# y00njaekim/CMU-11785-IDL-1.58bit-ASR

Hardware: AMD Instinct MI355X
Metric: mel-frames/sec (Conformer-S 1.58-bit train step) (higher is better)
Workload: dtype fp32; 1 GPU; conformer-s-1.58bit-train-step; global_batch=32, execution=hip-graph, per_gpu_batch=32, frames=1000, d_model=144, blocks=16, d_ff=576, heads=4, vocab=5004, parallelism=dp1, passes=teacher 2-bit + student 1-bit + SP, conv_pointwise=fp32 (reference)

## Files before the change

cmu-11785-idl-1.58bit-asr_amd/csrc/capi.hip:

```cpp
#include <float.h>

#include <algorithm>
#include <vector>

#include "../../include/onebit_hip.h"
#include "ob_launch.h"
#include <stdint.h>

using namespace ob;

namespace {

constexpr int kAbiVersion = 4;

inline hipStream_t as_stream(void* s) { return reinterpret_cast<hipStream_t>(s); }

inline bool aligned4(const void* p) { return (reinterpret_cast<uintptr_t>(p) & 3) == 0; }
inline bool misaligned8(const void* p) { return (reinterpret_cast<uintptr_t>(p) & 7) != 0; }

inline int check_bits(int bits) { return (bits == 1 || bits == 2) ? OB_OK : OB_ERR_BITWIDTH; }

inline int launched() {
  const hipError_t e = hipGetLastError();
  return e == hipSuccess ? OB_OK : OB_ERR_HIP;
// ... 2090 lines not shown
    return OB_ERR_NULL;
  if (((uintptr_t)saved & 15) || ((uintptr_t)probs & 15)) return OB_ERR_ALIGN;
  launch_relattn_fwd(q, k, v, pos, u, vb, lens, Bt, P, T, H, d, p_drop,
                     reinterpret_cast<const uint64_t*>(rng), (uint64_t)rng_offset, saved, probs,
                     ctx, as_stream(stream));
  return launched();
}

int64_t ob_relattn_saved_elems(int64_t Bt, int64_t T, int64_t H, int64_t d) {
  if (Bt < 1 || H < 1 || !relattn_supported(T, d)) return 0;
  return relattn_saved_elems(Bt, T, H, d);
}

size_t ob_relattn_bwd_workspace(int64_t Bt, int64_t T, int64_t H, int64_t d) {
  if (Bt < 1 || H < 1 || !relattn_supported(T, d)) return 0;
  return align_up(relattn_bwd_workspace(Bt, T, H, d));
}

int ob_relattn_set_bwd_mode(int mode) { return relattn_set_flash(mode); }

int ob_tgemm_set_colloop(int on) { return tgemm_set_colloop(on); }

int ob_relattn_set_kv_ring(int on) { return relattn_set_kv_ring(on); }

int64_t ob_relattn_probs_elems(int64_t Bt, int64_t T, int64_t H) {
  if (Bt < 1 || H < 1 || T < 1) return 0;
  return relattn_probs_elems(Bt, T, H);
}

int ob_relattn_bwd(const float* dctx, const float* ctx, const float* q, const float* k,
                   const float* v, const float* pos, const float* u, const float* vb,
                   const int32_t* lens, int64_t Bt, int64_t P, int64_t T, int64_t H, int64_t d,
                   float p_drop, const int64_t* rng, int64_t rng_offset, const float* saved,
                   int64_t saved_elems, float* dq, float* dk, float* dv, float* dpos, float* du,
                   float* dvb, void* ws, size_t ws_bytes, void* stream) {
  if (int st = relattn_check(Bt, P, T, H, d, p_drop)) return st;
  if (!dctx || !ctx || !q || !k || !v || !pos || !u || !vb || !lens || !saved || !dq || !dk ||
      !dv || !dpos || !du || !dvb || !ws)
    return OB_ERR_NULL;
  if (saved_elems != relattn_saved_elems(Bt, T, H, d)) return OB_ERR_SHAPE;
  (void)rng;
  (void)rng_offset;
  if ((uintptr_t)saved & 15) return OB_ERR_ALIGN;
  if (ws_bytes < ob_relattn_bwd_workspace(Bt, T, H, d)) return OB_ERR_WORKSPACE;
  launch_relattn_bwd(dctx, ctx, q, k, v, pos, u, vb, lens, Bt, P, T, H, d, p_drop, saved, dq, dk,
                     dv, dpos, du, dvb, ws, as_stream(stream));
// ... 107 lines not shown
```

cmu-11785-idl-1.58bit-asr_amd/csrc/ob_launch.h:

```cpp
#pragma once

#include <hip/hip_runtime.h>
#include <stddef.h>
#include <stdint.h>

#include "../../include/onebit_hip.h"

namespace ob {

inline int64_t ceil_div(int64_t a, int64_t b) { return (a + b - 1) / b; }

void launch_quant_pack(const float* W, const float* alpha, int alpha_raw, int bits,
                       const int* bits_dev, int64_t N, int64_t K, uint32_t* codes,
                       uint32_t* codes_t, hipStream_t s);
int64_t quant_pack_item_blocks(int64_t N, int64_t K);
int64_t quant_pack_item_blocks16(int64_t N, int64_t K);
void launch_quant_pack_group(const ob_pack_item* items_dev, int n_items, int64_t total_blocks,
                             hipStream_t s);
void launch_quant_dequant(const float* W, const float* alpha, int alpha_raw, int bits, int64_t n,
                          float* W_hat, hipStream_t s);

int64_t ste_reduce_blocks(int64_t total);
void launch_ste_reduce(const float* part, int chunks, int64_t nk, const float* part_db,
                       int64_t n_db, const float* W, const float* alpha, int alpha_raw, int bits,
// ... 438 lines not shown
  float* param;
  const float* grad;
  float* exp_avg;
  float* exp_avg_sq;
  int64_t numel;
};
int64_t adamw_plan(const int64_t* numels, int64_t n, int64_t* map);
size_t adamw_workspace(int64_t n_blocks);
void launch_adamw(const AdamwTensor* tab, const int64_t* map, int64_t nb, const float* lr,
                  float* step, float grad_scale, double beta1, double beta2, double eps,
                  double weight_decay, double max_norm, float* total_norm_out, void* ws,
                  hipStream_t s);

bool embed_supported(int64_t C);
void launch_embed_bwd(const int64_t* idx, int64_t N, const float* g, int64_t C, int64_t V,
                      int64_t pad, float* dW, hipStream_t s);

bool relattn_supported(int64_t T, int64_t d);
size_t relattn_bwd_workspace(int64_t Bt, int64_t T, int64_t H, int64_t d);
int64_t relattn_probs_elems(int64_t Bt, int64_t T, int64_t H);
int64_t relattn_saved_elems(int64_t Bt, int64_t T, int64_t H, int64_t d);
int relattn_set_flash(int on);
int relattn_set_kv_ring(int on);
void launch_relattn_fwd(const float* q, const float* k, const float* v, const float* pos,
                        const float* u, const float* vb, const int* lens, int64_t Bt, int64_t P,
                        int64_t T, int64_t H, int64_t d, float p_drop, const uint64_t* rng,
                        uint64_t rng_off, float* saved, float* probs, float* ctx, hipStream_t s);
void launch_relattn_bwd(const float* dctx, const float* ctx, const float* q, const float* k,
                        const float* v, const float* pos, const float* u, const float* vb,
                        const int* lens, int64_t Bt, int64_t P, int64_t T, int64_t H, int64_t d,
                        float p_drop, const float* saved, float* dq, float* dk, float* dv,
                        float* dpos, float* du, float* dvb, void* ws, hipStream_t s);
void launch_relattn_dropout_mask(int64_t n, int64_t T, float p_drop, const uint64_t* rng,
                                 uint64_t rng_off, uint8_t* out, hipStream_t s);

bool subsample_supported(int64_t T, int64_t F, int64_t C);
size_t subsample_image_bytes(int64_t C);
void launch_subsample_pack(const float* W2, int64_t C, void* img, hipStream_t s);
void launch_subsample_fwd(const float* X, int64_t B, int64_t T, int64_t F, int64_t C,
                          const float* W0, const float* b0, const void* img, const float* b2,
                          float* Y1, float* Y2, hipStream_t s);
size_t subsample_bwd_workspace(int64_t B, int64_t T, int64_t F, int64_t C);
void launch_subsample_bwd(const float* X, const float* W0, const float* b0, const float* Y1,
                          const float* Y2, const float* dY2, int64_t B, int64_t T, int64_t F,
                          int64_t C, const void* img,
                          float* dW0, float* db0, float* dW2, float* db2, void* ws,
// ... 4 lines not shown
```

cmu-11785-idl-1.58bit-asr_amd/csrc/relattn.hip:

```cpp
#include <atomic>
#include <math.h>

#include <algorithm>

#include "ob_drop.h"
#include "ob_launch.h"
#include "ob_mma.h"

namespace {
template <typename F>
__device__ __forceinline__ uint32_t xrows_1632(uint32_t x, F op) {
  const auto a = __builtin_amdgcn_permlane16_swap(x, x, false, false);
  x = op(a[0], a[1]);
  const auto b = __builtin_amdgcn_permlane32_swap(x, x, false, false);
  return op(b[0], b[1]);
}
__device__ __forceinline__ float xsum_1632(float v) {
  return __builtin_bit_cast(float, xrows_1632(__builtin_bit_cast(uint32_t, v), [](uint32_t a, uint32_t b) {
    return __builtin_bit_cast(uint32_t, __builtin_bit_cast(float, a) + __builtin_bit_cast(float, b));
  }));
}
__device__ __forceinline__ float xmax_1632(float v) {
  return __builtin_bit_cast(float, xrows_1632(__builtin_bit_cast(uint32_t, v), [](uint32_t a, uint32_t b) {
    return __builtin_bit_cast(uint32_t, fmaxf(__builtin_bit_cast(float, a), __builtin_bit_cast(float, b)));
  }));
}
__device__ __forceinline__ uint32_t xor_1632(uint32_t v) {
  return xrows_1632(v, [](uint32_t a, uint32_t b) { return a | b; });
}
}

namespace ob {

namespace {

constexpr int kThreads = 256;
constexpr int kTile = 64;
constexpr int kFwdKeyChunk = 256;

__device__ __forceinline__ void split_pair(float x0, float x1, uint32_t (&w)[3]) {
  __bf16 h0, m0, l0, h1, m1, l1;
  split3(x0, h0, m0, l0);
  split3(x1, h1, m1, l1);
  w[0] = (uint32_t)__builtin_bit_cast(uint16_t, h0) | ((uint32_t)__builtin_bit_cast(uint16_t, h1) << 16);
  w[1] = (uint32_t)__builtin_bit_cast(uint16_t, m0) | ((uint32_t)__builtin_bit_cast(uint16_t, m1) << 16);
  w[2] = (uint32_t)__builtin_bit_cast(uint16_t, l0) | ((uint32_t)__builtin_bit_cast(uint16_t, l1) << 16);
}

typedef f32x4 f32x4u __attribute__((aligned(4)));
template <int N>
__device__ __forceinline__ void load_run(const float* __restrict__ p, float (&out)[N]) {
#pragma unroll
  for (int i = 0; i + 4 <= N; i += 4) {
    const f32x4 v = *(const f32x4u*)(p + i);
    out[i] = v[0];
    out[i + 1] = v[1];
    out[i + 2] = v[2];
    out[i + 3] = v[3];
  }
#pragma unroll
  for (int i = N & ~3; i < N; ++i) out[i] = p[i];
// ... 12 lines not shown
  return __builtin_amdgcn_make_buffer_rsrc(const_cast<float*>(base), (short)0,
                                           (int)(((size_t)(T - 1) * C + D) * sizeof(float)),
                                           0x00020000);
}

template <int DQ>
__device__ __forceinline__ void load_group_buf(__amdgpu_buffer_rsrc_t rs, int voff, int C, int t0,
                                               float (&dst)[4][DQ]) {
#pragma unroll
  for (int u = 0; u < 4; ++u) {
    const int soff = 64 * (t0 + u) * C;
#pragma unroll
    for (int i = 0; i + 4 <= DQ; i += 4) {
      const f32x4 v = __builtin_amdgcn_raw_buffer_load_b128(rs, voff + 4 * i, soff, 0);
      dst[u][i] = v[0];
      dst[u][i + 1] = v[1];
      dst[u][i + 2] = v[2];
      dst[u][i + 3] = v[3];
    }
#pragma unroll
    for (int i = DQ & ~3; i < DQ; ++i)
      dst[u][i] = __builtin_bit_cast(float, __builtin_amdgcn_raw_buffer_load_b32(rs, voff + 4 * i, soff, 0));
  }
}

struct BlockId {
  int qt, h, b;
};

__device__ __forceinline__ BlockId block_id(int nqt, int H) {
  const int L = xcd_logical((int)blockIdx.x, (int)gridDim.x);
  BlockId id;
  id.qt = L % nqt;
  const int rest = L / nqt;
  id.h = rest % H;
  id.b = rest / H;
  return id;
}

__device__ __forceinline__ size_t frag_off(int bh, int a, int t, int nt) {
  return (((size_t)bh * nt + a) * nt + t) * 256;
}

__device__ __forceinline__ uint64_t drop_row_base(int bh, int T, int i) {
  return ((uint64_t)bh * T + i) * (uint64_t)(T + (T & 1));
}
// ... 13 lines not shown
      st_acc[k] += st_n - st_t;                              \
      st_t = st_n;                                           \
    }                                                        \
  } while (0)
#define OB_STAMP_WRITE(NWV)                                                             \
  if constexpr (st_on) {                                                                \
    const uint64_t st_rt1 = __builtin_amdgcn_s_memrealtime();                           \
    const size_t st_w = (size_t)blockIdx.x * (NWV) + w;                                 \
    if (lane == 0 && st_w * 10 + 10 <= 65536)                                           \
      for (int k_ = 0; k_ < 10; ++k_) g_attn_stamps[st_w * 10 + k_] = st_acc[k_];       \
    if (lane == 0 && st_w * 2 + 2 <= 16384) {                                           \
      g_attn_rt[st_w * 2] = st_rt0;                                                     \
      g_attn_rt[st_w * 2 + 1] = st_rt1;                                                 \
    }                                                                                   \
  }
#else
#define OB_STAMP_DECL(K)
#define OB_STAMP(k) \
  do {              \
  } while (0)
#define OB_STAMP_WRITE(NWV)
#endif

template <int DQ, int NTT>
__global__ __launch_bounds__(kThreads) void relattn_fwd_kernel(
    const float* __restrict__ q, const float* __restrict__ k, const float* __restrict__ v,
    const float* __restrict__ pos, const float* __restrict__ u, const float* __restrict__ vbias,
    const int* __restrict__ lens, int Bp, int T, int H, float inv_sqrt_d, DropCfg dc,
    const uint64_t* __restrict__ rng, uint64_t rng_off, float* __restrict__ probs,
    float* __restrict__ stats, uint32_t* __restrict__ kbits, float* __restrict__ anchors,
    float* __restrict__ ctx) {
  constexpr int D = 4 * DQ;
  constexpr int CT = (D + 15) / 16;
  extern __shared__ float img[];
  const int nt = (T + 15) >> 4;
  const int ldi = T + 1;
  const BlockId bid = block_id((T + kTile - 1) / kTile, H);
  const int b = bid.b, h = bid.h, i0 = bid.qt * kTile;
  const int bh = b * H + h;
  const int pass = b / Bp;
  const int C = H * D;
  const int L = min(lens[b], T);
  const int lane = threadIdx.x & 63, w = threadIdx.x >> 6, r = lane & 15, g = lane >> 4;
  const float* qb = q + (size_t)b * T * C + h * D;
  const float* kb = k + (size_t)b * T * C + h * D;
  const float* vbp = v + (size_t)b * T * C + h * D;
  const float* pb = pos + (size_t)pass * T * C + h * D;
  const float* ub = u + h * D;
  const float* vbb = vbias + h * D;
  const __amdgpu_buffer_rsrc_t rs_p = slice_rsrc(pb, T, C, D), rs_k = slice_rsrc(kb, T, C, D);
  const int voff_a = (r * C + g * DQ) * 4;
  OB_STAMP_DECL(3)

  const int ir = 16 * w + r;
  const int qi = i0 + ir;
  const int qic = min(qi, T - 1);
  float qu[DQ], qv[DQ];
  {
    float x[DQ];
    load_run<DQ>(qb + (size_t)qic * C + g * DQ, x);
#pragma unroll
    for (int s = 0; s < DQ; ++s) {
      const int c = g * DQ + s;
      qu[s] = x[s] + ub[c];
      qv[s] = x[s] + vbb[c];
    }
  }

  float opb[2][4][DQ];
  load_group_buf<DQ>(rs_p, voff_a, C, 0, opb[0]);
  OB_STAMP(0);
#pragma unroll
  for (int t0 = 0; t0 < NTT; t0 += 4) {
    if (t0 >= nt) continue;
    float (&opa)[4][DQ] = opb[(t0 >> 2) & 1];
    if (t0 + 4 < NTT && t0 + 4 < nt) load_group_buf<DQ>(rs_p, voff_a, C, t0 + 4, opb[((t0 >> 2) + 1) & 1]);
    f32x4 acc[4];
#pragma unroll
    for (int uu = 0; uu < 4; ++uu) acc[uu] = f32x4{0.f, 0.f, 0.f, 0.f};
#pragma unroll
    for (int s = 0; s < DQ; ++s)
#pragma unroll
      for (int uu = 0; uu < 4; ++uu) acc[uu] = mfma4(opa[uu][s], qv[s], acc[uu]);
#pragma unroll
    for (int uu = 0; uu < 4; ++uu) {
      const int t = t0 + uu;
      if (t >= nt) continue;
      float* dst = img + ir * ldi + 1 + 16 * t + 4 * g;
      if (16 * t + 15 < T) {
#pragma unroll
        for (int j = 0; j < 4; ++j) dst[j] = acc[uu][j];
      } else {
#pragma unroll
        for (int j = 0; j < 4; ++j)
          if (16 * t + 4 * g + j < T) dst[j] = acc[uu][j];
      }
    }
  }
  if (g == 0) img[ir * ldi] = 0.0f;
  OB_STAMP(1);
  load_group_buf<DQ>(rs_k, voff_a, C, 0, opb[0]);
  if (i0 + kTile < T) {
    const float* qe = qb + (size_t)(i0 + kTile) * C;
    for (int m = threadIdx.x; m < T; m += kThreads) {
      float pr[D];
      load_run<D>(pb + (size_t)m * C, pr);
      float a = 0.0f;
#pragma unroll
      for (int c = 0; c < D; ++c) a = fmaf(qe[c] + vbb[c], pr[c], a);
      img[kTile * ldi + 1 + m] = a;
    }
    if (threadIdx.x == 0) img[kTile * ldi] = 0.0f;
  }
  OB_STAMP(2);
  __syncthreads();
  OB_STAMP(3);
  if (anchors) {
    const int nchk = (16 * nt + 31) / 32;
#pragma unroll
    for (int half = 0; half < 2; ++half) {
      const int row = i0 + 32 * half;
      if (row < 32 || row >= T) continue;
      float* dst = anchors + ((size_t)bh * nchk + row / 32 - 1) * T;
      for (int m = threadIdx.x; m < T; m += kThreads) dst[m] = img[32 * half * ldi + 1 + m];
    }
  }

  float sreg[NTT][4];
  float mx = -INFINITY;
  const float* bdp = img + (T + ir * T + 4 * g - i0);
  const int Lq = qi < L ? L : 0;
#pragma unroll
  for (int t0 = 0; t0 < NTT; t0 += 4) {
    if (t0 >= nt) continue;
    float (&opa)[4][DQ] = opb[(t0 >> 2) & 1];
    if (t0 + 4 < NTT && t0 + 4 < nt) load_group_buf<DQ>(rs_k, voff_a, C, t0 + 4, opb[((t0 >> 2) + 1) & 1]);
    f32x4 acc4[4];
#pragma unroll
    for (int uu = 0; uu < 4; ++uu) acc4[uu] = f32x4{0.f, 0.f, 0.f, 0.f};
#pragma unroll
    for (int s = 0; s < DQ; ++s)
#pragma unroll
      for (int uu = 0; uu < 4; ++uu) acc4[uu] = mfma4(opa[uu][s], qu[s], acc4[uu]);
#pragma unroll
    for (int uu = 0; uu < 4; ++uu) {
      const int t = t0 + uu;
      if (t >= nt) continue;
#pragma unroll
      for (int j = 0; j < 4; ++j) {
        const float sc = (acc4[uu][j] + bdp[16 * t + j]) * inv_sqrt_d;
        sreg[t][j] = 16 * t + 4 * g + j < Lq ? sc : -INFINITY;
        mx = fmaxf(mx, sreg[t][j]);
      }
    }
  }
  mx = xmax_1632(mx);
  OB_STAMP(4);
  constexpr int kVSlots = (kFwdKeyChunk / 2 * DQ + kThreads - 1) / kThreads;
  constexpr bool kVPre = DQ <= 9;
// ... 149 lines not shown
          for (int j = 0; j < 4; ++j) {
            bfr[p][j] = lo[j];
            bfr[p][4 + j] = hi[j];
          }
        }
        o[ct] = mfma_x6(af, bfr, o[ct]);
      }
    }
  }
#pragma unroll
  for (int ct = 0; ct < CT; ++ct) {
    const int col = 16 * ct + r;
    if (col >= D) continue;
#pragma unroll
    for (int j = 0; j < 4; ++j) {
      const int row = i0 + 16 * w + 4 * g + j;
      if (row < T) ctx[((size_t)b * T + row) * C + h * D + col] = o[ct][j];
    }
  }
  OB_STAMP(9);
  OB_STAMP_WRITE(kThreads / 64)
}

template <int DQ, int NTT>
__global__ __launch_bounds__(kThreads) void relattn_bwd_kernel(
    const float* __restrict__ dctx, const float* __restrict__ ctxo, const float* __restrict__ k,
    const float* __restrict__ v, const float* __restrict__ pos, int Bp, int T, int H,
    float inv_sqrt_d, DropCfg dc, const float* __restrict__ probs, float* __restrict__ dq,
    float* __restrict__ dsg, float* __restrict__ du_part, float* __restrict__ dvb_part) {
  constexpr int D = 4 * DQ;
  constexpr int CT = (D + 15) / 16;
  extern __shared__ float band[];
  __shared__ float red[kThreads / 64][2][64];
  const int nt = (T + 15) >> 4;
  const int nqt = (T + kTile - 1) / kTile;
  const BlockId bid = block_id(nqt, H);
  const int b = bid.b, h = bid.h, qt = bid.qt, i0 = qt * kTile;
  const int bh = b * H + h;
  const int pass = b / Bp;
  const int C = H * D;
  const int lane = threadIdx.x & 63, w = threadIdx.x >> 6, r = lane & 15, g = lane >> 4;
  const size_t bo = (size_t)b * T * C + h * D;
  const float* kb = k + bo;
  const float* vbp = v + bo;
  const float* dob = dctx + bo;
  const float* cob = ctxo + bo;
  const float* pb = pos + (size_t)pass * T * C + h * D;
  const __amdgpu_buffer_rsrc_t rs_v = slice_rsrc(vbp, T, C, D), rs_k = slice_rsrc(kb, T, C, D),
                               rs_p = slice_rsrc(pb, T, C, D);
  const int voff_a = (r * C + g * DQ) * 4;
  auto keep_scale = [&](float pv) -> float {
    if (!dc.on) return 1.0f;
    return __builtin_signbit(pv) ? 0.0f : dc.scale;
  };
  if (threadIdx.x < 128) band[(kTile + 1) * T + threadIdx.x] = 0.0f;
  OB_STAMP_DECL(2)

  const int ir = 16 * w + r;
  const int qi = i0 + ir;
  const int qic = min(qi, T - 1);
  float dor[DQ];
  load_run<DQ>(dob + (size_t)qic * C + g * DQ, dor);
  float delta;
  {
    float cr[DQ];
    load_run<DQ>(cob + (size_t)qic * C + g * DQ, cr);
    float a = 0.0f;
#pragma unroll
    for (int s = 0; s < DQ; ++s) a = fmaf(dor[s], cr[s], a);
    a = xsum_1632(a);
    delta = a;
  }
  OB_STAMP(0);

  const bool arow_ok = (i0 >> 4) + w < nt;
  const float* pf = probs + frag_off(bh, arow_ok ? (i0 >> 4) + w : 0, 0, nt) + 4 * lane;
  float* brow = band + (1 + ir) * T + 4 * g;
  float dsr[NTT][4];
  float opb[2][4][DQ];
  load_group_buf<DQ>(rs_v, voff_a, C, 0, opb[0]);
#pragma unroll
  for (int t0 = 0; t0 < NTT; t0 += 4) {
    if (t0 >= nt) continue;
    float (&opa)[4][DQ] = opb[(t0 >> 2) & 1];
    if (t0 + 4 < NTT && t0 + 4 < nt) load_group_buf<DQ>(rs_v, voff_a, C, t0 + 4, opb[((t0 >> 2) + 1) & 1]);
    f32x4 p4[4];
#pragma unroll
    for (int uu = 0; uu < 4; ++uu)
      p4[uu] = arow_ok && t0 + uu < nt ? *reinterpret_cast<const f32x4*>(pf + 256 * (t0 + uu))
                                       : f32x4{0.f, 0.f, 0.f, 0.f};
    f32x4 acc4[4];
#pragma unroll
    for (int uu = 0; uu < 4; ++uu) acc4[uu] = f32x4{0.f, 0.f, 0.f, 0.f};
#pragma unroll
    for (int s = 0; s < DQ; ++s)
#pragma unroll
      for (int uu = 0; uu < 4; ++uu) acc4[uu] = mfma4(opa[uu][s], dor[s], acc4[uu]);
#pragma unroll
    for (int uu = 0; uu < 4; ++uu) {
      const int t = t0 + uu;
      if (t >= nt) continue;
#pragma unroll
      for (int j = 0; j < 4; ++j) {
        const float pv = p4[uu][j];
        const float dp = acc4[uu][j] * keep_scale(pv);
        const float ds = (fabsf(pv) * (dp - delta)) * inv_sqrt_d;
        dsr[t][j] = ds;
      }
      if (16 * t + 15 < T) {
#pragma unroll
        for (int j = 0; j < 4; ++j) brow[16 * t + j] = dsr[t][j];
      } else {
#pragma unroll
        for (int j = 0; j < 4; ++j)
          if (16 * t + 4 * g + j < T) brow[16 * t + j] = dsr[t][j];
      }
    }
  }

  OB_STAMP(1);
  if (i0 > 0) {
    const int ip = i0 - 1;
    const float* drow = dob + (size_t)ip * C;
    const float* crow = cob + (size_t)ip * C;
    float dl = 0.0f;
#pragma unroll
    for (int c = 0; c < D; ++c) dl = fmaf(drow[c], crow[c], dl);
    const float* pr = probs + frag_off(bh, ip >> 4, 0, nt) + 4 * (ip & 15);
    for (int jj = threadIdx.x; jj < T; jj += kThreads) {
      float vr[D];
      load_run<D>(vbp + (size_t)jj * C, vr);
      float a = 0.0f;
#pragma unroll
      for (int c = 0; c < D; ++c) a = fmaf(vr[c], drow[c], a);
      const float pv = pr[256 * (jj >> 4) + 64 * ((jj & 15) >> 2) + (jj & 3)];
      band[jj] = (fabsf(pv) * (a * keep_scale(pv) - dl)) * inv_sqrt_d;
    }
  } else {
    for (int jj = threadIdx.x; jj < T; jj += kThreads) band[jj] = 0.0f;
  }
  OB_STAMP(2);

  f32x4 oq[CT];
#pragma unroll
  for (int ct = 0; ct < CT; ++ct) oq[ct] = f32x4{0.f, 0.f, 0.f, 0.f};
  const int voff_b = (4 * g * C + r) * 4;
  auto load_b = [&](int t, float (&dst)[4][CT]) {
#pragma unroll
    for (int j = 0; j < 4; ++j)
#pragma unroll
      for (int ct = 0; ct < CT; ++ct)
        dst[j][ct] = __builtin_bit_cast(float, __builtin_amdgcn_raw_buffer_load_b32(
                                                   rs_k, voff_b + 4 * (j * C + 16 * ct), 64 * t * C, 0));
  };
  {
    float kbb[2][4][CT];
    load_b(0, kbb[0]);
#pragma unroll
    for (int t = 0; t < NTT; ++t) {
      if (t >= nt) continue;
      if (t + 1 < NTT && t + 1 < nt) load_b(t + 1, kbb[(t + 1) & 1]);
#pragma unroll
      for (int j = 0; j < 4; ++j)
#pragma unroll
        for (int ct = 0; ct < CT; ++ct) oq[ct] = mfma4(dsr[t][j], kbb[t & 1][j][ct], oq[ct]);
    }
  }
  OB_STAMP(3);
  __syncthreads();
  OB_STAMP(4);

  f32x4 ov[CT];
#pragma unroll
  for (int ct = 0; ct < CT; ++ct) ov[ct] = f32x4{0.f, 0.f, 0.f, 0.f};
  const float* xrow = band + i0 + 1 + ir * (T + 1) + g;
  const int nk = (T + 3) >> 2;
  constexpr int kMK = 8;
  const int voff_pm = (g * C + r) * 4;
  auto load_p = [&](int mk0, float (&dst)[kMK][CT]) {
#pragma unroll
    for (int qq = 0; qq < kMK; ++qq)
#pragma unroll
      for (int ct = 0; ct < CT; ++ct)
        dst[qq][ct] = __builtin_bit_cast(float, __builtin_amdgcn_raw_buffer_load_b32(
                                                    rs_p, voff_pm + 64 * ct, 16 * (mk0 + qq) * C, 0));
  };
  float pv_cur[kMK][CT];
  load_p(0, pv_cur);
  for (int mk0 = 0; mk0 < nk; mk0 += kMK) {
    float pv_nxt[kMK][CT];
    if (mk0 + kMK < nk) load_p(mk0 + kMK, pv_nxt);
#pragma unroll
    for (int qq = 0; qq < kMK; ++qq) {
      const float av = mk0 + qq < nk ? xrow[4 * (mk0 + qq)] : 0.0f;
#pragma unroll
      for (int ct = 0; ct < CT; ++ct) ov[ct] = mfma4(av, pv_cur[qq][ct], ov[ct]);
    }
#pragma unroll
    for (int qq = 0; qq < kMK; ++qq)
#pragma unroll
      for (int ct = 0; ct < CT; ++ct) pv_cur[qq][ct] = pv_nxt[qq][ct];
  }
  OB_STAMP(5);
  float su[CT], sv[CT];
#pragma unroll
  for (int ct = 0; ct < CT; ++ct) {
    const int col = 16 * ct + r;
    su[ct] = 0.0f;
    sv[ct] = 0.0f;
#pragma unroll
    for (int j = 0; j < 4; ++j) {
      const int row = i0 + 16 * w + 4 * g + j;
      if (row < T) {
        su[ct] += oq[ct][j];
        sv[ct] += ov[ct][j];
        if (col < D) dq[bo + (size_t)row * C + col] = oq[ct][j] + ov[ct][j];
      }
    }
    su[ct] = xsum_1632(su[ct]);
    sv[ct] = xsum_1632(sv[ct]);
  }
  const size_t tile_id = ((size_t)b * H + h) * nqt + qt;
#pragma unroll
  for (int ct = 0; ct < CT; ++ct) {
// ... 1017 lines not shown
  int m = g_flash.load(std::memory_order_relaxed);
  if (m < 0) {
    const char* e = getenv("OB_ATTN_BWD");
    int want = (e != nullptr && e[0] == 'f') ? 1 : 0;
    g_flash.compare_exchange_strong(m, want);
    m = g_flash.load(std::memory_order_relaxed);
  }
  return m == 1;
}
int relattn_set_flash(int on) {
  const int prev = flash_selected() ? 1 : 0;
  if (on == 0 || on == 1) g_flash.store(on, std::memory_order_relaxed);
  return prev;
}
bool relattn_fused(int64_t T, int64_t d) { return T <= 256 && d <= 36 && flash_selected(); }

static std::atomic<int> g_kv_ring{1};
int relattn_set_kv_ring(int on) {
  const int prev = g_kv_ring.load(std::memory_order_relaxed);
  if (on == 0 || on == 1) g_kv_ring.store(on, std::memory_order_relaxed);
  return prev;
}

struct SavedLayout {
  int64_t stats, kbits, tail, total;
  SavedLayout(int64_t Bt, int64_t T, int64_t H, int64_t d) {
    const int64_t nt = (T + 15) / 16, Tp = 16 * nt, W = (nt + 1) / 2, nch = (Tp + 31) / 32;
    stats = 0;
    kbits = Bt * H * Tp * 2;
    tail = kbits + Bt * H * Tp * W;
    tail = (tail + 3) & ~(int64_t)3;
    total = tail + (relattn_fused(T, d) ? Bt * H * nch * T : relattn_probs_elems(Bt, T, H));
  }
};

int64_t relattn_saved_elems(int64_t Bt, int64_t T, int64_t H, int64_t d) {
  return SavedLayout(Bt, T, H, d).total;
}

int64_t relattn_probs_elems(int64_t Bt, int64_t T, int64_t H) {
  const int64_t nt = (T + 15) / 16;
  return Bt * H * nt * nt * 256;
}

int fused_splits(int64_t T) { return ((16 * ((T + 15) / 16) + 31) / 32) >= 2 ? 2 : 1; }

// ... 15 lines not shown
    } else if (d == 32) {                      \
      if (big) KERNEL(8, 32); else KERNEL(8, 16);   \
    } else if (d == 36) {                      \
      if (big) KERNEL(9, 32); else KERNEL(9, 16);   \
    } else {                                   \
      if (big) KERNEL(16, 32); else KERNEL(16, 16); \
    }                                          \
  } while (0)

void launch_relattn_fwd(const float* q, const float* k, const float* v, const float* pos,
                        const float* u, const float* vb, const int* lens, int64_t Bt, int64_t P,
                        int64_t T, int64_t H, int64_t d, float p_drop, const uint64_t* rng,
                        uint64_t rng_off, float* saved, float* probs, float* ctx, hipStream_t s) {
  const dim3 grid((unsigned)(((T + kTile - 1) / kTile) * H * Bt));
  const DropCfg dc = make_drop(p_drop);
  const float inv_sqrt_d = 1.0f / (float)sqrt((double)d);
  const size_t lds = fwd_lds_bytes((int)T, (int)d);
  const SavedLayout sl(Bt, T, H, d);
  const bool flash = saved && relattn_fused(T, d);
  float* stats = flash ? saved : nullptr;
  uint32_t* kbits = flash ? reinterpret_cast<uint32_t*>(saved + sl.kbits) : nullptr;
  float* anchors = flash ? saved + sl.tail : nullptr;
  if (saved && !relattn_fused(T, d)) probs = saved + sl.tail;
#define OB_RA_FWD(DQ, NTT)                                                                 \
  hipLaunchKernelGGL((relattn_fwd_kernel<DQ, NTT>), grid, dim3(kThreads), lds, s, q, k, v, pos, \
                     u, vb, lens, (int)(Bt / P), (int)T, (int)H, inv_sqrt_d, dc, rng, rng_off, probs, \
                     stats, kbits, anchors, ctx)
  OB_RA_DISPATCH(OB_RA_FWD);
#undef OB_RA_FWD
}

constexpr int kFusedWaves = 8;

void launch_relattn_bwd(const float* dctx, const float* ctx, const float* q, const float* k,
                        const float* v, const float* pos, const float* u, const float* vb,
                        const int* lens, int64_t Bt, int64_t P, int64_t T, int64_t H, int64_t d,
                        float p_drop, const float* saved, float* dq, float* dk, float* dv,
                        float* dpos, float* du, float* dvb, void* ws, hipStream_t s) {
  const int64_t nt = (T + 15) / 16, Tp = 16 * nt, W = (nt + 1) / 2;
  if (relattn_fused(T, d)) {
    const DropCfg dc = make_drop(p_drop);
    const float inv_sqrt_d = 1.0f / (float)sqrt((double)d);
    const int ns = fused_splits(T);
    const int64_t C = H * d;
    const int64_t n_kv = Bt * T * C;
    float* dp_part = (float*)ws;
    float* du_part = dp_part + (size_t)Bt * H * ns * T * d;
    float* dvb_part = du_part + (size_t)Bt * H * ns * d;
    float* kv_part = dvb_part + (size_t)Bt * H * ns * d;
    kv_part += (16 - ((uintptr_t)kv_part & 15)) / 4 % 4;
    const SavedLayout sl(Bt, T, H, d);
    const float* stats = saved;
// ... 11 lines not shown
    if (d == 16) OB_RA_FUSED(4);
    else if (d == 32) OB_RA_FUSED(8);
    else OB_RA_FUSED(9);
#undef OB_RA_FUSED
    const int n_dpos = (int)ceil_div(P * T * C, 64);
    const int n_bias = (int)(2 * H * ((d + kBiasCols - 1) / kBiasCols));
    const int n_kvb = ns > 1 ? (int)ceil_div(2 * n_kv, 4 * kThreads) : 0;
    hipLaunchKernelGGL(relattn_reduce_kernel, dim3((unsigned)(n_dpos + n_bias + n_kvb)),
                       dim3(kThreads), 0, s, (const float*)dp_part, (const float*)du_part,
                       (const float*)dvb_part, (int)Bt, (int)P, (int)T, (int)H, (int)d, ns, n_dpos,
                       dpos, du, dvb, ns, n_bias, (const float*)kv_part, n_kv, dk, dv);
    return;
  }
  const float* probs = saved + SavedLayout(Bt, T, H, d).tail;
  const int nqt = (int)((T + kTile - 1) / kTile);
  const dim3 grid((unsigned)(nqt * H * Bt));
  const DropCfg dc = make_drop(p_drop);
  const float inv_sqrt_d = 1.0f / (float)sqrt((double)d);
  const size_t lds = bwd_lds_bytes((int)T);
  float* dsg = (float*)ws;
  float* dp_part = dsg + (size_t)Bt * H * T * T;
  float* du_part = dp_part + (size_t)Bt * H * T * d;
  float* dvb_part = du_part + (size_t)Bt * H * nqt * d;
#define OB_RA_BWD(DQ, NTT)                                                                     \
  hipLaunchKernelGGL((relattn_bwd_kernel<DQ, NTT>), grid, dim3(kThreads), lds, s, dctx, ctx, k,    \
                     v, pos, (int)(Bt / P), (int)T, (int)H, inv_sqrt_d, dc, probs, dq, dsg,        \
                     du_part, dvb_part)
  OB_RA_DISPATCH(OB_RA_BWD);
#undef OB_RA_BWD
  const bool ring = g_kv_ring.load(std::memory_order_relaxed) == 1;
#define OB_RA_KV(DQ, NTT)                                                                          \
  do {                                                                                             \
    if (ring)                                                                                      \
      hipLaunchKernelGGL((relattn_bwd_kv_ring_kernel<DQ>), grid, dim3(kThreads), 0, s,              \
                         (const float*)dsg, probs, q, dctx, u, vb, (int)T, (int)H, dc, dk, dv,      \
                         dp_part);                                                                 \
    else                                                                                           \
      hipLaunchKernelGGL((relattn_bwd_kv_kernel<DQ>), grid, dim3(kThreads), 0, s,                   \
                         (const float*)dsg, probs, q, dctx, u, vb, (int)T, (int)H, dc, dk, dv,      \
                         dp_part);                                                                 \
  } while (0)
  OB_RA_DISPATCH(OB_RA_KV);
#undef OB_RA_KV
  const int64_t C = H * d;
  const int n_dpos = (int)ceil_div(P * T * C, 64);
  const int n_bias = (int)(2 * H * ((d + kBiasCols - 1) / kBiasCols));
  hipLaunchKernelGGL(relattn_reduce_kernel, dim3((unsigned)(n_dpos + n_bias)), dim3(kThreads), 0, s,
                     (const float*)dp_part, (const float*)du_part, (const float*)dvb_part, (int)Bt,
                     (int)P, (int)T, (int)H, (int)d, nqt, n_dpos, dpos, du, dvb, 1, n_bias,
                     (const float*)nullptr, (int64_t)0, (float*)nullptr, (float*)nullptr);
}

// ... 18 lines not shown
```

cmu-11785-idl-1.58bit-asr_amd/onebit_asr/_lib.py:

```python
from __future__ import annotations

import ctypes
import os
from pathlib import Path

import torch

LIB_NAME = "libonebit_hip.so"
LIB_PATH = Path(os.environ.get("ONEBIT_HIP_LIB") or Path(__file__).with_name(LIB_NAME))

OB_OK = 0
OB_ERR_SHAPE = -2
OB_ERR_BITWIDTH = -3

_c_f = ctypes.c_void_p
_i64 = ctypes.c_int64
_int = ctypes.c_int
_sz = ctypes.c_size_t
_f32 = ctypes.c_float
_f64 = ctypes.c_double

SIGNATURES = {
    "ob_abi_version": (_int, []),
    "ob_source_digest": (ctypes.c_char_p, []),
# ... 232 lines not shown
               _f32, _c_f, _i64, _c_f, _c_f, _c_f]),
    "ob_bitlinear_bwd_dx_passes": (
        _int, [_c_f, _i64, _i64, _i64, _c_f, _c_f, _c_f, _c_f, _int, _i64, _c_f, _c_f]),
    "ob_bitlinear_bwd_dw_passes_workspace": (_sz, [_i64, _i64, _i64, _i64]),
    "ob_bitlinear_bwd_dw_passes": (
        _int, [_c_f, _c_f, _i64, _i64, _i64, _i64, _c_f, _c_f, _int, _c_f, _c_f, _c_f, _c_f, _c_f,
               _sz, _c_f]),
    "ob_bitlinear_bwd_dw_passes_group_workspace": (_sz, [_i64, _i64, _i64, _i64, _i64]),
    "ob_bitlinear_bwd_dw_passes_group": (
        _int, [_i64, _c_f, _c_f, _i64, _i64, _i64, _i64, _c_f, _c_f, _int, _c_f, _c_f, _c_f, _c_f,
               _c_f, _sz, _c_f]),
    "ob_relattn_fwd": (
        _int, [_c_f, _c_f, _c_f, _c_f, _c_f, _c_f, _c_f, _i64, _i64, _i64, _i64, _i64, _f32, _c_f,
               _i64, _c_f, _c_f, _c_f, _c_f]),
    "ob_relattn_saved_elems": (_i64, [_i64, _i64, _i64, _i64]),
    "ob_relattn_probs_elems": (_i64, [_i64, _i64, _i64]),
    "ob_relattn_bwd_workspace": (_sz, [_i64, _i64, _i64, _i64]),
    "ob_relattn_bwd": (
        _int, [_c_f, _c_f, _c_f, _c_f, _c_f, _c_f, _c_f, _c_f, _c_f, _i64, _i64, _i64, _i64, _i64,
               _f32, _c_f, _i64, _c_f, _i64, _c_f, _c_f, _c_f, _c_f, _c_f, _c_f, _c_f, _sz, _c_f]),
    "ob_relattn_set_bwd_mode": (_int, [_int]),
    "ob_tgemm_set_colloop": (_int, [_int]),
    "ob_relattn_set_kv_ring": (_int, [_int]),
    "ob_relattn_dropout_mask": (_int, [_i64, _i64, _f32, _c_f, _i64, _c_f, _c_f]),
    "ob_embedding_bwd": (_int, [_c_f, _i64, _c_f, _i64, _i64, _i64, _c_f, _c_f]),
    "ob_adamw_plan": (_i64, [_c_f, _i64, _c_f]),
    "ob_adamw_workspace": (_sz, [_i64]),
    "ob_adamw_clip_step": (
        _int, [_c_f, _i64, _c_f, _i64, _c_f, _c_f, _f32, _f64, _f64, _f64, _f64, _f64, _c_f, _c_f,
               _sz, _c_f]),
}

ABI_VERSION = 4

_lib = None


class OneBitHipError(RuntimeError):
    pass


def load() -> ctypes.CDLL:
    global _lib
    if _lib is not None:
        return _lib
    if not LIB_PATH.is_file():
# ... 64 lines not shown
```

include/onebit_hip.h:

```cpp
#ifndef ONEBIT_HIP_H_
#define ONEBIT_HIP_H_

#include <stddef.h>
#include <stdint.h>

#ifdef __cplusplus
extern "C" {
#endif

#define OB_API __attribute__((visibility("default")))

enum {
  OB_OK = 0,
  OB_ERR_NULL = -1,
  OB_ERR_SHAPE = -2,
  OB_ERR_BITWIDTH = -3,
  OB_ERR_WORKSPACE = -4,
  OB_ERR_ALIGN = -5,
  OB_ERR_HIP = -6
};

OB_API int ob_abi_version(void);
OB_API const char* ob_source_digest(void);
OB_API const char* ob_status_string(int status);
// ... 212 lines not shown
OB_API int ob_decattn_fwd_grouped(const float* q, int64_t sq, const float* k, int64_t sk,
                                  const float* v, int64_t sv, const uint8_t* kmask,
                                  int64_t causal, int64_t B, int64_t kv_group, int64_t H,
                                  int64_t Lq, int64_t Lk, int64_t dh, float* ctx, void* stream);

OB_API int ob_relattn_fwd(const float* q, const float* k, const float* v, const float* pos,
                          const float* u, const float* vb, const int32_t* lens, int64_t Bt,
                          int64_t P, int64_t T, int64_t H, int64_t d, float p_drop,
                          const int64_t* rng, int64_t rng_offset, float* saved, float* probs,
                          float* ctx, void* stream);
OB_API int64_t ob_relattn_saved_elems(int64_t Bt, int64_t T, int64_t H, int64_t d);
OB_API int64_t ob_relattn_probs_elems(int64_t Bt, int64_t T, int64_t H);
OB_API size_t ob_relattn_bwd_workspace(int64_t Bt, int64_t T, int64_t H, int64_t d);
OB_API int ob_relattn_bwd(const float* dctx, const float* ctx, const float* q, const float* k,
                          const float* v, const float* pos, const float* u, const float* vb,
                          const int32_t* lens, int64_t Bt, int64_t P, int64_t T, int64_t H,
                          int64_t d, float p_drop, const int64_t* rng, int64_t rng_offset,
                          const float* saved, int64_t saved_elems,
                          float* dq, float* dk, float* dv, float* dpos, float* du, float* dvb,
                          void* ws, size_t ws_bytes, void* stream);
OB_API int ob_relattn_set_bwd_mode(int mode);
OB_API int ob_tgemm_set_colloop(int on);
OB_API int ob_relattn_set_kv_ring(int on);
OB_API int ob_relattn_dropout_mask(int64_t n, int64_t row_len, float p_drop, const int64_t* rng,
                                   int64_t rng_offset, uint8_t* out, void* stream);

OB_API int ob_embedding_bwd(const int64_t* indices, int64_t N, const float* grad, int64_t C,
                            int64_t V, int64_t padding_idx, float* grad_weight, void* stream);

typedef struct ob_adamw_tensor {
  float* param;
  const float* grad;
  float* exp_avg;
  float* exp_avg_sq;
  int64_t numel;
} ob_adamw_tensor;

OB_API int64_t ob_adamw_plan(const int64_t* numels, int64_t n_tensors, int64_t* chunk_map);
OB_API size_t ob_adamw_workspace(int64_t n_blocks);
OB_API int ob_adamw_clip_step(const ob_adamw_tensor* table, int64_t n_tensors,
                              const int64_t* chunk_map, int64_t n_blocks, const float* lr,
                              float* step, float grad_scale, double beta1, double beta2,
                              double eps, double weight_decay, double max_norm,
                              float* total_norm, void* ws,
                              size_t ws_bytes, void* stream);

// ... 305 lines not shown
```

Baseline: 1.443 million mel-frames/s.

## Add full-window relattn kernel variants with deeper prefetch and scheduling fences

Adds a WIN template specialization to the relative-attention forward and backward kernels. It applies when T rounds exactly to the compiled tile count (NTT), so bounds checks become compile-time and loads can be software-pipelined with sched_barrier fences. The backward variant prefetches probability fragments ahead, triple-buffers the K operand loads and double-buffers the PV loop. It is enabled by default through a runtime mask, and the cost is extra registers (occupancy risk) and more kernel instantiations.

```diff
diff --git a/cmu-11785-idl-1.58bit-asr_amd/csrc/capi.hip b/cmu-11785-idl-1.58bit-asr_amd/csrc/capi.hip
--- a/cmu-11785-idl-1.58bit-asr_amd/csrc/capi.hip
+++ b/cmu-11785-idl-1.58bit-asr_amd/csrc/capi.hip
@@ -2136,6 +2136,7 @@
 int ob_tgemm_set_colloop(int on) { return tgemm_set_colloop(on); }
 
 int ob_relattn_set_kv_ring(int on) { return relattn_set_kv_ring(on); }
+int ob_relattn_set_windows(int mask) { return relattn_set_windows(mask); }
 
 int64_t ob_relattn_probs_elems(int64_t Bt, int64_t T, int64_t H) {
   if (Bt < 1 || H < 1 || T < 1) return 0;
diff --git a/cmu-11785-idl-1.58bit-asr_amd/csrc/ob_launch.h b/cmu-11785-idl-1.58bit-asr_amd/csrc/ob_launch.h
--- a/cmu-11785-idl-1.58bit-asr_amd/csrc/ob_launch.h
+++ b/cmu-11785-idl-1.58bit-asr_amd/csrc/ob_launch.h
@@ -484,6 +484,7 @@
 int64_t relattn_saved_elems(int64_t Bt, int64_t T, int64_t H, int64_t d);
 int relattn_set_flash(int on);
 int relattn_set_kv_ring(int on);
+int relattn_set_windows(int mask);
 void launch_relattn_fwd(const float* q, const float* k, const float* v, const float* pos,
                         const float* u, const float* vb, const int* lens, int64_t Bt, int64_t P,
                         int64_t T, int64_t H, int64_t d, float p_drop, const uint64_t* rng,
diff --git a/cmu-11785-idl-1.58bit-asr_amd/csrc/relattn.hip b/cmu-11785-idl-1.58bit-asr_amd/csrc/relattn.hip
--- a/cmu-11785-idl-1.58bit-asr_amd/csrc/relattn.hip
+++ b/cmu-11785-idl-1.58bit-asr_amd/csrc/relattn.hip
@@ -2,6 +2,7 @@
 #include <math.h>
 
 #include <algorithm>
+#include <type_traits>
 
 #include "ob_drop.h"
 #include "ob_launch.h"
@@ -37,6 +38,10 @@
 constexpr int kThreads = 256;
 constexpr int kTile = 64;
 constexpr int kFwdKeyChunk = 256;
+#ifndef OB_ATTN_WIN_PAHEAD
+#define OB_ATTN_WIN_PAHEAD 1
+#endif
+constexpr int kWinPAhead = OB_ATTN_WIN_PAHEAD;
 
 __device__ __forceinline__ void split_pair(float x0, float x1, uint32_t (&w)[3]) {
   __bf16 h0, m0, l0, h1, m1, l1;
@@ -95,6 +100,11 @@
     for (int i = DQ & ~3; i < DQ; ++i)
       dst[u][i] = __builtin_bit_cast(float, __builtin_amdgcn_raw_buffer_load_b32(rs, voff + 4 * i, soff, 0));
   }
+}
+
+template <bool WIN>
+__device__ __forceinline__ void win_fence() {
+  if constexpr (WIN) __builtin_amdgcn_sched_barrier(0);
 }
 
 struct BlockId {
@@ -154,7 +164,7 @@
 #define OB_STAMP_WRITE(NWV)
 #endif
 
-template <int DQ, int NTT>
+template <int DQ, int NTT, bool WIN = false>
 __global__ __launch_bounds__(kThreads) void relattn_fwd_kernel(
     const float* __restrict__ q, const float* __restrict__ k, const float* __restrict__ v,
     const float* __restrict__ pos, const float* __restrict__ u, const float* __restrict__ vbias,
@@ -165,7 +175,7 @@
   constexpr int D = 4 * DQ;
   constexpr int CT = (D + 15) / 16;
   extern __shared__ float img[];
-  const int nt = (T + 15) >> 4;
+  const int nt = WIN ? NTT : (T + 15) >> 4;
   const int ldi = T + 1;
   const BlockId bid = block_id((T + kTile - 1) / kTile, H);
   const int b = bid.b, h = bid.h, i0 = bid.qt * kTile;
@@ -206,7 +216,9 @@
   for (int t0 = 0; t0 < NTT; t0 += 4) {
     if (t0 >= nt) continue;
     float (&opa)[4][DQ] = opb[(t0 >> 2) & 1];
+    win_fence<WIN>();
     if (t0 + 4 < NTT && t0 + 4 < nt) load_group_buf<DQ>(rs_p, voff_a, C, t0 + 4, opb[((t0 >> 2) + 1) & 1]);
+    win_fence<WIN>();
     f32x4 acc[4];
 #pragma unroll
     for (int uu = 0; uu < 4; ++uu) acc[uu] = f32x4{0.f, 0.f, 0.f, 0.f};
@@ -219,7 +231,7 @@
       const int t = t0 + uu;
       if (t >= nt) continue;
       float* dst = img + ir * ldi + 1 + 16 * t + 4 * g;
-      if (16 * t + 15 < T) {
+      if ((WIN && t < NTT - 1) || 16 * t + 15 < T) {
 #pragma unroll
         for (int j = 0; j < 4; ++j) dst[j] = acc[uu][j];
       } else {
@@ -266,7 +278,9 @@
   for (int t0 = 0; t0 < NTT; t0 += 4) {
     if (t0 >= nt) continue;
     float (&opa)[4][DQ] = opb[(t0 >> 2) & 1];
+    win_fence<WIN>();
     if (t0 + 4 < NTT && t0 + 4 < nt) load_group_buf<DQ>(rs_k, voff_a, C, t0 + 4, opb[((t0 >> 2) + 1) & 1]);
+    win_fence<WIN>();
     f32x4 acc4[4];
 #pragma unroll
     for (int uu = 0; uu < 4; ++uu) acc4[uu] = f32x4{0.f, 0.f, 0.f, 0.f};
@@ -462,7 +476,7 @@
   OB_STAMP_WRITE(kThreads / 64)
 }
 
-template <int DQ, int NTT>
+template <int DQ, int NTT, bool WIN = false>
 __global__ __launch_bounds__(kThreads) void relattn_bwd_kernel(
     const float* __restrict__ dctx, const float* __restrict__ ctxo, const float* __restrict__ k,
     const float* __restrict__ v, const float* __restrict__ pos, int Bp, int T, int H,
@@ -472,7 +486,7 @@
   constexpr int CT = (D + 15) / 16;
   extern __shared__ float band[];
   __shared__ float red[kThreads / 64][2][64];
-  const int nt = (T + 15) >> 4;
+  const int nt = WIN ? NTT : (T + 15) >> 4;
   const int nqt = (T + kTile - 1) / kTile;
   const BlockId bid = block_id(nqt, H);
   const int b = bid.b, h = bid.h, qt = bid.qt, i0 = qt * kTile;
@@ -513,22 +527,37 @@
   }
   OB_STAMP(0);
 
-  const bool arow_ok = (i0 >> 4) + w < nt;
+  const bool arow_ok = WIN || (i0 >> 4) + w < nt;
   const float* pf = probs + frag_off(bh, arow_ok ? (i0 >> 4) + w : 0, 0, nt) + 4 * lane;
   float* brow = band + (1 + ir) * T + 4 * g;
   float dsr[NTT][4];
   float opb[2][4][DQ];
   load_group_buf<DQ>(rs_v, voff_a, C, 0, opb[0]);
+  f32x4 pq[WIN ? NTT : 1];
+  constexpr int kPA = 4 * kWinPAhead;
+  if constexpr (WIN) {
+#pragma unroll
+    for (int t = 0; t < kPA && t < NTT; ++t) pq[t] = *reinterpret_cast<const f32x4*>(pf + 256 * t);
+    win_fence<WIN>();
+  }
 #pragma unroll
   for (int t0 = 0; t0 < NTT; t0 += 4) {
     if (t0 >= nt) continue;
     float (&opa)[4][DQ] = opb[(t0 >> 2) & 1];
+    win_fence<WIN>();
     if (t0 + 4 < NTT && t0 + 4 < nt) load_group_buf<DQ>(rs_v, voff_a, C, t0 + 4, opb[((t0 >> 2) + 1) & 1]);
     f32x4 p4[4];
-#pragma unroll
-    for (int uu = 0; uu < 4; ++uu)
-      p4[uu] = arow_ok && t0 + uu < nt ? *reinterpret_cast<const f32x4*>(pf + 256 * (t0 + uu))
-                                       : f32x4{0.f, 0.f, 0.f, 0.f};
+    if constexpr (WIN) {
+#pragma unroll
+      for (int uu = 0; uu < 4; ++uu)
+        if (t0 + kPA + uu < NTT) pq[t0 + kPA + uu] = *reinterpret_cast<const f32x4*>(pf + 256 * (t0 + kPA + uu));
+      win_fence<WIN>();
+    } else {
+#pragma unroll
+      for (int uu = 0; uu < 4; ++uu)
+        p4[uu] = arow_ok && t0 + uu < nt ? *reinterpret_cast<const f32x4*>(pf + 256 * (t0 + uu))
+                                         : f32x4{0.f, 0.f, 0.f, 0.f};
+    }
     f32x4 acc4[4];
 #pragma unroll
     for (int uu = 0; uu < 4; ++uu) acc4[uu] = f32x4{0.f, 0.f, 0.f, 0.f};
@@ -536,6 +565,10 @@
     for (int s = 0; s < DQ; ++s)
 #pragma unroll
       for (int uu = 0; uu < 4; ++uu) acc4[uu] = mfma4(opa[uu][s], dor[s], acc4[uu]);
+    if constexpr (WIN) {
+#pragma unroll
+      for (int uu = 0; uu < 4; ++uu) p4[uu] = pq[t0 + uu];
+    }
 #pragma unroll
     for (int uu = 0; uu < 4; ++uu) {
       const int t = t0 + uu;
@@ -547,7 +580,7 @@
         const float ds = (fabsf(pv) * (dp - delta)) * inv_sqrt_d;
         dsr[t][j] = ds;
       }
-      if (16 * t + 15 < T) {
+      if ((WIN && t < NTT - 1) || 16 * t + 15 < T) {
 #pragma unroll
         for (int j = 0; j < 4; ++j) brow[16 * t + j] = dsr[t][j];
       } else {
@@ -593,7 +626,21 @@
         dst[j][ct] = __builtin_bit_cast(float, __builtin_amdgcn_raw_buffer_load_b32(
                                                    rs_k, voff_b + 4 * (j * C + 16 * ct), 64 * t * C, 0));
   };
-  {
+  if constexpr (WIN) {
+    float kbb[3][4][CT];
+    load_b(0, kbb[0]);
+    load_b(1, kbb[1]);
+#pragma unroll
+    for (int t = 0; t < NTT; ++t) {
+      win_fence<WIN>();
+      if (t + 2 < NTT) load_b(t + 2, kbb[(t + 2) % 3]);
+      win_fence<WIN>();
+#pragma unroll
+      for (int j = 0; j < 4; ++j)
+#pragma unroll
+        for (int ct = 0; ct < CT; ++ct) oq[ct] = mfma4(dsr[t][j], kbb[t % 3][j][ct], oq[ct]);
+    }
+  } else {
     float kbb[2][4][CT];
     load_b(0, kbb[0]);
 #pragma unroll
@@ -625,6 +672,37 @@
         dst[qq][ct] = __builtin_bit_cast(float, __builtin_amdgcn_raw_buffer_load_b32(
                                                     rs_p, voff_pm + 64 * ct, 16 * (mk0 + qq) * C, 0));
   };
+  if constexpr (WIN) {
+    constexpr int NR = NTT / 2;
+    float pvb[2][kMK][CT], avb[2][kMK];
+    auto load_x = [&](int rd, float (&dst)[kMK]) {
+#pragma unroll
+      for (int qq = 0; qq < kMK; ++qq) {
+        const int mk = kMK * rd + qq;
+        if (rd + 1 < NR) {
+          dst[qq] = xrow[4 * mk];
+        } else {
+          const float x = xrow[4 * min(mk, nk - 1)];
+          dst[qq] = mk < nk ? x : 0.0f;
+        }
+      }
+    };
+    load_p(0, pvb[0]);
+    load_x(0, avb[0]);
+#pragma unroll
+    for (int rd = 0; rd < NR; ++rd) {
+      win_fence<WIN>();
+      if (rd + 1 < NR) {
+        load_p(kMK * (rd + 1), pvb[(rd + 1) & 1]);
+        load_x(rd + 1, avb[(rd + 1) & 1]);
+      }
+      win_fence<WIN>();
+#pragma unroll
+      for (int qq = 0; qq < kMK; ++qq)
+#pragma unroll
+        for (int ct = 0; ct < CT; ++ct) ov[ct] = mfma4(avb[rd & 1][qq], pvb[rd & 1][qq][ct], ov[ct]);
+    }
+  } else {
   float pv_cur[kMK][CT];
   load_p(0, pv_cur);
   for (int mk0 = 0; mk0 < nk; mk0 += kMK) {
@@ -640,6 +718,7 @@
     for (int qq = 0; qq < kMK; ++qq)
 #pragma unroll
       for (int ct = 0; ct < CT; ++ct) pv_cur[qq][ct] = pv_nxt[qq][ct];
+  }
   }
   OB_STAMP(5);
   float su[CT], sv[CT];
@@ -1703,6 +1782,18 @@
   return prev;
 }
 
+static std::atomic<int> g_windows{3};
+int relattn_set_windows(int mask) {
+  const int prev = g_windows.load(std::memory_order_relaxed);
+  if (mask >= 0 && mask <= 3) g_windows.store(mask, std::memory_order_relaxed);
+  return prev;
+}
+constexpr bool win_built(int DQ, int NTT) { return !(DQ == 16 && NTT == 32); }
+static bool windows_on(int bit, int64_t T, int64_t d) {
+  return ((g_windows.load(std::memory_order_relaxed) >> bit) & 1) &&
+         (T + 15) / 16 == (T > 256 ? 32 : 16) && win_built(d == 64 ? 16 : 0, T > 256 ? 32 : 16);
+}
+
 struct SavedLayout {
   int64_t stats, kbits, tail, total;
   SavedLayout(int64_t Bt, int64_t T, int64_t H, int64_t d) {
@@ -1764,12 +1855,25 @@
   uint32_t* kbits = flash ? reinterpret_cast<uint32_t*>(saved + sl.kbits) : nullptr;
   float* anchors = flash ? saved + sl.tail : nullptr;
   if (saved && !relattn_fused(T, d)) probs = saved + sl.tail;
-#define OB_RA_FWD(DQ, NTT)                                                                 \
-  hipLaunchKernelGGL((relattn_fwd_kernel<DQ, NTT>), grid, dim3(kThreads), lds, s, q, k, v, pos, \
-                     u, vb, lens, (int)(Bt / P), (int)T, (int)H, inv_sqrt_d, dc, rng, rng_off, probs, \
-                     stats, kbits, anchors, ctx)
+#define OB_RA_FWD_W(DQ, NTT, WIN)                                                               \
+  hipLaunchKernelGGL((relattn_fwd_kernel<DQ, NTT, WIN>), grid, dim3(kThreads), lds, s, q, k, v,   \
+                     pos, u, vb, lens, (int)(Bt / P), (int)T, (int)H, inv_sqrt_d, dc, rng, rng_off, \
+                     probs, stats, kbits, anchors, ctx)
+  const bool win = windows_on(1, T, d);
+  auto launch = [&](auto dq_c, auto ntt_c) {
+    constexpr int DQ = decltype(dq_c)::value, NTT = decltype(ntt_c)::value;
+    if constexpr (win_built(DQ, NTT)) {
+      if (win) {
+        OB_RA_FWD_W(DQ, NTT, true);
+        return;
+      }
+    }
+    OB_RA_FWD_W(DQ, NTT, false);
+  };
+#define OB_RA_FWD(DQ, NTT) launch(std::integral_constant<int, DQ>{}, std::integral_constant<int, NTT>{})
   OB_RA_DISPATCH(OB_RA_FWD);
 #undef OB_RA_FWD
+#undef OB_RA_FWD_W
 }
 
 constexpr int kFusedWaves = 8;
@@ -1827,12 +1931,25 @@
   float* dp_part = dsg + (size_t)Bt * H * T * T;
   float* du_part = dp_part + (size_t)Bt * H * T * d;
   float* dvb_part = du_part + (size_t)Bt * H * nqt * d;
-#define OB_RA_BWD(DQ, NTT)                                                                     \
-  hipLaunchKernelGGL((relattn_bwd_kernel<DQ, NTT>), grid, dim3(kThreads), lds, s, dctx, ctx, k,    \
-                     v, pos, (int)(Bt / P), (int)T, (int)H, inv_sqrt_d, dc, probs, dq, dsg,        \
+#define OB_RA_BWD_W(DQ, NTT, WIN)                                                                \
+  hipLaunchKernelGGL((relattn_bwd_kernel<DQ, NTT, WIN>), grid, dim3(kThreads), lds, s, dctx, ctx,  \
+                     k, v, pos, (int)(Bt / P), (int)T, (int)H, inv_sqrt_d, dc, probs, dq, dsg,     \
                      du_part, dvb_part)
+  const bool win = windows_on(0, T, d);
+  auto launch = [&](auto dq_c, auto ntt_c) {
+    constexpr int DQ = decltype(dq_c)::value, NTT = decltype(ntt_c)::value;
+    if constexpr (win_built(DQ, NTT)) {
+      if (win) {
+        OB_RA_BWD_W(DQ, NTT, true);
+        return;
+      }
+    }
+    OB_RA_BWD_W(DQ, NTT, false);
+  };
+#define OB_RA_BWD(DQ, NTT) launch(std::integral_constant<int, DQ>{}, std::integral_constant<int, NTT>{})
   OB_RA_DISPATCH(OB_RA_BWD);
 #undef OB_RA_BWD
+#undef OB_RA_BWD_W
   const bool ring = g_kv_ring.load(std::memory_order_relaxed) == 1;
 #define OB_RA_KV(DQ, NTT)                                                                          \
   do {                                                                                             \
diff --git a/cmu-11785-idl-1.58bit-asr_amd/onebit_asr/_lib.py b/cmu-11785-idl-1.58bit-asr_amd/onebit_asr/_lib.py
--- a/cmu-11785-idl-1.58bit-asr_amd/onebit_asr/_lib.py
+++ b/cmu-11785-idl-1.58bit-asr_amd/onebit_asr/_lib.py
@@ -278,6 +278,7 @@
     "ob_relattn_set_bwd_mode": (_int, [_int]),
     "ob_tgemm_set_colloop": (_int, [_int]),
     "ob_relattn_set_kv_ring": (_int, [_int]),
+    "ob_relattn_set_windows": (_int, [_int]),
     "ob_relattn_dropout_mask": (_int, [_i64, _i64, _f32, _c_f, _i64, _c_f, _c_f]),
     "ob_embedding_bwd": (_int, [_c_f, _i64, _c_f, _i64, _i64, _i64, _c_f, _c_f]),
     "ob_adamw_plan": (_i64, [_c_f, _i64, _c_f]),
diff --git a/include/onebit_hip.h b/include/onebit_hip.h
--- a/include/onebit_hip.h
+++ b/include/onebit_hip.h
@@ -258,6 +258,7 @@
 OB_API int ob_relattn_set_bwd_mode(int mode);
 OB_API int ob_tgemm_set_colloop(int on);
 OB_API int ob_relattn_set_kv_ring(int on);
+OB_API int ob_relattn_set_windows(int mask);
 OB_API int ob_relattn_dropout_mask(int64_t n, int64_t row_len, float p_drop, const int64_t* rng,
                                    int64_t rng_offset, uint8_t* out, void* stream);
 
```

Measured after the change: 1.467 million mel-frames/s, median of 6. 1.7% higher.
